# theovincent/iS-DQN

Hardware: AMD Instinct MI355X
Metric: gradient-steps/sec (batch=256, K=9, 84x84x4) (higher is better)
Workload: dtype bf16x3 (split-bf16 MFMA operands hi+lo, fp32 accumulate)

## Files before the change

is-dqn_amd/csrc/gemm_core.h:

```cpp
#pragma once
#include <cstdio>
#include <cstdlib>
#include <type_traits>
#include "common.h"

namespace isdqn {

typedef __attribute__((ext_vector_type(8))) __bf16 bf16x8;
typedef __attribute__((ext_vector_type(4))) short s16x4;
typedef __attribute__((ext_vector_type(8))) short s16x8;
typedef __attribute__((ext_vector_type(4))) float f32x4;

constexpr int GEMM_BK = 32;
constexpr int GEMM_THREADS = 256;

__device__ __forceinline__ int xcd_remap(int bid, int n_blocks) {
    const int xcd = bid & 7, q = n_blocks >> 3, r = n_blocks & 7;
    const int base = xcd < r ? xcd * (q + 1) : r * (q + 1) + (xcd - r) * q;
    return base + (bid >> 3);
}

#define LDS_AS __attribute__((address_space(3)))

__device__ __forceinline__ void split8(const float (&v)[8], bf16x8& hi, bf16x8& lo) {
// ... 86 lines not shown
    return ((chunk >> 4) << 2) + (((chunk >> 2) & 1) << 1) + ((chunk >> 3) & 1);
}
__device__ __forceinline__ constexpr int tr_row(int kk) {
    return 16 * (kk >> 4) + 8 * ((kk >> 2) & 1) + 2 * (kk & 3) + ((kk >> 3) & 1);
}
template <int ROWS, bool TR, int TR_PAD = 16>
struct TileGeom {
    static constexpr int PITCH = TR ? (ROWS + TR_PAD) : (GEMM_BK + 16);
    static constexpr int ELEMS = TR ? GEMM_BK * PITCH : ROWS * PITCH;
    static constexpr int CHUNKS = ROWS * (GEMM_BK / 8);
    static constexpr int PER_THREAD = (CHUNKS + GEMM_THREADS - 1) / GEMM_THREADS;
};

__device__ __forceinline__ void mfma_init(f32x4& acc) { acc = f32x4{0.f, 0.f, 0.f, 0.f}; }
__device__ __forceinline__ void mfma_acc(f32x4& acc, const bf16x8& a, const bf16x8& b) {
    acc = __builtin_amdgcn_mfma_f32_16x16x32_bf16(a, b, acc, 0, 0, 0);
}

template <bool TR, int PITCH>
__device__ __forceinline__ bf16x8 read_frag(const __bf16* tile, int row0, int lane) {
    if constexpr (!TR) {
        return *reinterpret_cast<const bf16x8*>(tile + (row0 + (lane & 15)) * PITCH + (lane >> 4) * 8);
    } else {
        const int g = lane >> 4, i = lane & 15, q = i >> 2, p = i & 3;
        const __bf16* a0 = tile + (16 * (g >> 1) + 2 * q + (g & 1)) * PITCH + row0 + 4 * p;
        const __bf16* a1 = a0 + 8 * PITCH;
        s16x4 lo = __builtin_amdgcn_ds_read_tr16_b64_v4i16((LDS_AS s16x4*)a0);
        s16x4 hi = __builtin_amdgcn_ds_read_tr16_b64_v4i16((LDS_AS s16x4*)a1);
        s16x8 r = __builtin_shufflevector(lo, hi, 0, 1, 2, 3, 4, 5, 6, 7);
        return __builtin_bit_cast(bf16x8, r);
    }
}

template <class P, class = void>
struct KGroupsOf { static constexpr int value = 1; };
template <class P>
struct KGroupsOf<P, std::void_t<decltype(P::KG)>> { static constexpr int value = P::KG; };
template <class P, class = void>
struct TrPadAOf { static constexpr int value = 16; };
template <class P>
struct TrPadAOf<P, std::void_t<decltype(P::TR_PAD_A)>> { static constexpr int value = P::TR_PAD_A; };
template <class P, class = void>
struct TrPadBOf { static constexpr int value = 16; };
template <class P>
struct TrPadBOf<P, std::void_t<decltype(P::TR_PAD_B)>> { static constexpr int value = P::TR_PAD_B; };
template <class P, class = void>
struct AS8Of { static constexpr bool value = false; };
template <class P>
struct AS8Of<P, std::void_t<decltype(P::A_S8)>> { static constexpr bool value = P::A_S8; };
template <class P, class = void>
struct BS8Of { static constexpr bool value = false; };
template <class P>
struct BS8Of<P, std::void_t<decltype(P::B_S8)>> { static constexpr bool value = P::B_S8; };

template <class P>
struct GemmTraits {
    static constexpr int BM = P::BM, BN = P::BN, WM = P::WM, WN = P::WN;
    static constexpr int MT = BM / WM / 16, NT = BN / WN / 16;
    static constexpr int PASSES = P::PASSES;
    static constexpr int A_PLANES = PASSES >= 2 ? 2 : 1;
    static constexpr int B_PLANES = PASSES >= 3 ? 2 : 1;
    using GA = TileGeom<BM, P::A_TR, TrPadAOf<P>::value>;
    using GB = TileGeom<BN, P::B_TR, TrPadBOf<P>::value>;
    static constexpr int STAGE_ELEMS = A_PLANES * GA::ELEMS + B_PLANES * GB::ELEMS;
    static constexpr int KG = KGroupsOf<P>::value;
    static constexpr int PIPE_BYTES = KG * 2 * STAGE_ELEMS * 2;
    static constexpr int XCHG_BYTES = KG > 1 ? KG * 4 * NT * 4 * 64 * 4 : 0;
    static constexpr int EPI_BYTES = P::EPI_LDS_BYTES + XCHG_BYTES;
    static constexpr int LDS_BYTES = PIPE_BYTES > EPI_BYTES ? PIPE_BYTES : EPI_BYTES;
};

template <class P>
__global__ __launch_bounds__(GEMM_THREADS * KGroupsOf<P>::value) void gemm_kernel(const P p) {
    ISDQN_EMPTY_KERNEL_RETURN
    using T = GemmTraits<P>;
    constexpr int KG = T::KG;
    using GA = typename T::GA;
    using GB = typename T::GB;
    constexpr int MT = T::MT, NT = T::NT, PASSES = T::PASSES;
    extern __shared__ __attribute__((aligned(16))) char smem_raw[];
    __bf16* smem = reinterpret_cast<__bf16*>(smem_raw);

    typename P::Tile tile;
    if (!p.tile((int)blockIdx.x, tile)) return;

    const int kg = KG > 1 ? (int)threadIdx.x / GEMM_THREADS : 0;
    const int tid = (int)threadIdx.x - kg * GEMM_THREADS;
    const int lane = tid & 63;
    const int wave = tid >> 6;
    const int wm = wave / P::WN, wn = wave % P::WN;
    const int wave_m = wm * (MT * 16), wave_n = wn * (NT * 16);

    typename P::ACtx actx[GA::PER_THREAD];
    typename P::BCtx bctx[GB::PER_THREAD];
    int a_lds[GA::PER_THREAD], a_var[GA::PER_THREAD];
    int b_lds[GB::PER_THREAD], b_var[GB::PER_THREAD];
    bool a_on[GA::PER_THREAD], b_on[GB::PER_THREAD];
#pragma unroll
    for (int i = 0; i < GA::PER_THREAD; ++i) {
        int c = tid + i * GEMM_THREADS;
        a_on[i] = c < GA::CHUNKS;
        if (!a_on[i]) c = 0;
        if constexpr (!P::A_TR) {
            int r = stash_row(c), kc = c & 3;
            actx[i] = p.a_ctx(tile, tile.m0 + r);
            a_var[i] = kc * 8;
            a_lds[i] = r * GA::PITCH + kc * 8;
        } else {
            int kk = c / (T::BM / 8), rc = c % (T::BM / 8);
            actx[i] = p.a_ctx(tile, tile.m0 + rc * 8);
            a_var[i] = kk;
            a_lds[i] = tr_row(kk) * GA::PITCH + rc * 8;
        }
    }
#pragma unroll
    for (int i = 0; i < GB::PER_THREAD; ++i) {
        int c = tid + i * GEMM_THREADS;
        b_on[i] = c < GB::CHUNKS;
        if (!b_on[i]) c = 0;
        if constexpr (!P::B_TR) {
            int r = stash_row(c), kc = c & 3;
            bctx[i] = p.b_ctx(tile, tile.n0 + r);
            b_var[i] = kc * 8;
            b_lds[i] = r * GB::PITCH + kc * 8;
        } else {
            int kk = c / (T::BN / 8), rc = c % (T::BN / 8);
            bctx[i] = p.b_ctx(tile, tile.n0 + rc * 8);
            b_var[i] = kk;
            b_lds[i] = tr_row(kk) * GB::PITCH + rc * 8;
        }
    }

    float sa[GA::PER_THREAD][8], sb[GB::PER_THREAD][8];

    auto fetch = [&](int k) {
#pragma unroll
        for (int i = 0; i < GA::PER_THREAD; ++i)
// ... 31 lines not shown
                chunk_hi<BS8Of<P>::value>(sb[i], hi);
            }
            *reinterpret_cast<bf16x8*>(b_hi + b_lds[i]) = hi;
        }
    };

    f32x4 acc[MT][NT];
#pragma unroll
    for (int mt = 0; mt < MT; ++mt)
#pragma unroll
        for (int nt = 0; nt < NT; ++nt) mfma_init(acc[mt][nt]);

    auto compute = [&](int stage) {
        const __bf16* base = smem + (kg * 2 + stage) * T::STAGE_ELEMS;
        const __bf16* a_hi = base;
        const __bf16* a_lo = base + GA::ELEMS;
        const __bf16* b_hi = base + T::A_PLANES * GA::ELEMS;
        const __bf16* b_lo = b_hi + GB::ELEMS;
        bf16x8 fa_hi[MT], fa_lo[MT];
#pragma unroll
        for (int mt = 0; mt < MT; ++mt) {
            fa_hi[mt] = read_frag<P::A_TR, GA::PITCH>(a_hi, wave_m + mt * 16, lane);
            if constexpr (PASSES >= 2) fa_lo[mt] = read_frag<P::A_TR, GA::PITCH>(a_lo, wave_m + mt * 16, lane);
        }
#pragma unroll
        for (int nt = 0; nt < NT; ++nt) {
            bf16x8 fb_hi = read_frag<P::B_TR, GB::PITCH>(b_hi, wave_n + nt * 16, lane);
            bf16x8 fb_lo;
            if constexpr (PASSES >= 3) fb_lo = read_frag<P::B_TR, GB::PITCH>(b_lo, wave_n + nt * 16, lane);
#pragma unroll
            for (int mt = 0; mt < MT; ++mt) {
                if constexpr (PASSES >= 3)
                    mfma_acc(acc[mt][nt], fa_hi[mt], fb_lo);
                if constexpr (PASSES >= 2)
                    mfma_acc(acc[mt][nt], fa_lo[mt], fb_hi);
                mfma_acc(acc[mt][nt], fa_hi[mt], fb_hi);
            }
        }
    };

    const int nsteps = ((tile.k1 - tile.k0 + GEMM_BK - 1) / GEMM_BK + KG - 1) / KG;
    if (nsteps > 0) {
        fetch(tile.k0 + kg * GEMM_BK);
        stash(0);
        __syncthreads();
        for (int s = 0; s < nsteps; ++s) {
            const bool more = s + 1 < nsteps;
            if (more) fetch(tile.k0 + ((s + 1) * KG + kg) * GEMM_BK);
            compute(s & 1);
            if (more) stash((s + 1) & 1);
            __syncthreads();
        }
    }
    if constexpr (KG > 1) {
        static_assert(KG == 2 && MT == 2, "one row tile per K group");
        float* red = reinterpret_cast<float*>(smem_raw + P::EPI_LDS_BYTES);
#pragma unroll
        for (int nt = 0; nt < NT; ++nt)
#pragma unroll
            for (int r = 0; r < 4; ++r) {
                const float give = kg == 0 ? acc[1][nt][r] : acc[0][nt][r];
                red[(((kg * 4 + wave) * NT + nt) * 4 + r) * 64 + lane] = give;
            }
        __syncthreads();
        f32x4 mine[1][NT];
#pragma unroll
        for (int nt = 0; nt < NT; ++nt)
#pragma unroll
            for (int r = 0; r < 4; ++r) {
                const float got = red[((((1 - kg) * 4 + wave) * NT + nt) * 4 + r) * 64 + lane];
                mine[0][nt][r] = (kg == 0 ? acc[0][nt][r] : acc[1][nt][r]) + got;
            }
        p.epilogue(tile, mine, tile.m0 + wave_m + kg * 16, tile.n0 + wave_n, lane, smem_raw);
    } else {
        p.epilogue(tile, acc, tile.m0 + wave_m, tile.n0 + wave_n, lane, smem_raw);
    }
}

template <class P>
static int launch_gemm(const P& p, int n_blocks, hipStream_t stream) {
    using T = GemmTraits<P>;
    static LdsConfigured configured;
    int rc = ensure_dynamic_lds(&gemm_kernel<P>, T::LDS_BYTES, configured);
    if (rc) return rc;
    ISDQN_REPORT_OCCUPANCY((&gemm_kernel<P>), GEMM_THREADS * T::KG, T::LDS_BYTES, n_blocks);
    if (n_blocks <= 0) return ISDQN_OK;
    hipLaunchKernelGGL(gemm_kernel<P>, dim3(n_blocks), dim3(GEMM_THREADS * T::KG), T::LDS_BYTES, stream, p);
    ISDQN_HIP_CHECK(hipGetLastError());
    return ISDQN_OK;
}

__device__ __forceinline__ void zero8(float (&v)[8]) {
#pragma unroll
    for (int i = 0; i < 8; ++i) v[i] = 0.f;
}
__device__ __forceinline__ float row16_sum(float x) {
    auto dpp = [](float v, auto ctrl) {
        return __builtin_bit_cast(float, __builtin_amdgcn_update_dpp(0, __builtin_bit_cast(int, v), decltype(ctrl)::value, 0xF, 0xF, true));
    };
    x += dpp(x, std::integral_constant<int, 0xB1>{});
    x += dpp(x, std::integral_constant<int, 0x4E>{});
    x += dpp(x, std::integral_constant<int, 0x124>{});
    x += dpp(x, std::integral_constant<int, 0x128>{});
    return x;
}

// ... 85 lines not shown
```

is-dqn_amd/csrc/head_chain.h:

```cpp
#pragma once
struct HeadChainParams {
    const float* slabs;
    int n_slabs;
    int64_t slab_stride, row_pitch;
    const float* hbias;
    float* act;
    float* z;
    const float* W;
    const float* bias;
    const float* gamma;
    const float* beta;
    int B, S, F, Fp, O, Op, K, A, oh;
    const int* action;
    const float* reward;
    const uint8_t* terminal;
    const float* loss_weights;
    const float* discount;
    float gamma_n, huber_delta;
    int double_q;
    Munchausen mu;
    float* dout;
    float* dz;
    float* part;
    float* q_values;
    float* targets;
    double* priorities;
    float* loss_part;
    float* dbh_part;
    int* adam_count;
    float b1, b2;
    float* adam_consts;
    long long* stamps;
};

constexpr int HC_MAX_COLS = 4;
constexpr int HC_THREADS = 512, HC_WAVES = HC_THREADS / 64;
constexpr int HC_KU = 16 / HC_WAVES;

__host__ __device__ inline int head_chain_pitch(int Fp) { return (Fp + 31) / 32 * 32 + 8; }
static inline int head_chain_lds_bytes(int Fp, int Op, int K, int passes, int S) {
    const int PA = head_chain_pitch(Fp);
    return (passes >= 2 ? 2 : 1) * 16 * PA * 2 + (HC_WAVES * 16 * Op + 16 * Op + S * Op + Op + 4 + 2 * S * Fp) * 4 + S * K * 12 +
           HC_WAVES * 2 * S * 2 * 4 + 64;
}

template <int PASSES, int COLS, int SMAX>
__global__ __launch_bounds__(HC_THREADS) void head_chain_kernel(const HeadChainParams p) {
    ISDQN_EMPTY_KERNEL_RETURN
    extern __shared__ __attribute__((aligned(16))) char hc_smem[];
    const int PA = head_chain_pitch(p.Fp);
    constexpr int A_PLANES = PASSES >= 2 ? 2 : 1;
    __bf16* a_hi = reinterpret_cast<__bf16*>(hc_smem);
    __bf16* a_lo = a_hi + 16 * PA;
    float* qpart = reinterpret_cast<float*>(a_hi + A_PLANES * 16 * PA);
    float* s_q = qpart + HC_WAVES * 16 * p.Op;
    float* s_dq = s_q + 16 * p.Op;
    float* s_d = s_dq + SMAX * p.Op;
    float* s_td = s_d + SMAX * p.K;
    float* s_wtd = s_td + SMAX * p.K;
    float* s_red = s_wtd + SMAX * p.K;
    float* s_bias = s_red + HC_WAVES * 2 * SMAX * 2;
// ... 7 lines not shown
        if ((i) == 0) p.stamps[(int64_t)blockIdx.x * 8 + 7] = (long long)__builtin_amdgcn_s_memrealtime(); \
    }
#else
#define HC_STAMP(i)
#endif
    HC_STAMP(0);
    const int S = p.S, b0 = (int)blockIdx.x * S;
    const int Fp = p.Fp, Op = p.Op, K = p.K, A = p.A;

    if (blockIdx.x == 0 && tid == 0) {
        int t = *p.adam_count + 1;
        *p.adam_count = t;
        p.adam_consts[0] = (float)(1.0 - pow_int((double)p.b1, t));
        p.adam_consts[1] = (float)(1.0 - pow_int((double)p.b2, t));
    }

    int act[SMAX];
#pragma unroll
    for (int s = 0; s < SMAX; ++s) {
        ISDQN_BOUNDS_CHECK((s < S && b0 + s < p.B) ? (const void*)(p.action + b0 + s) : zero_chunk(), 4, 20);
        act[s] = *(const ISDQN_GLOBAL int*)((s < S && b0 + s < p.B) ? (const void*)(p.action + b0 + s) : zero_chunk());
    }
    float td_r, td_w, td_g;
    uint8_t td_term;
    {
        const int s = tid / K;
        const bool ok = tid < S * K && b0 + s < p.B;
        const bool okw = ok && p.loss_weights != nullptr;
        ISDQN_BOUNDS_CHECK(okw ? (const void*)(p.loss_weights + b0 + s) : zero_chunk(), 4, 29);
        td_w = *(const ISDQN_GLOBAL float*)(okw ? (const void*)(p.loss_weights + b0 + s) : zero_chunk());
        const bool okg = ok && p.discount != nullptr;
        ISDQN_BOUNDS_CHECK(okg ? (const void*)(p.discount + b0 + s) : zero_chunk(), 4, 50);
        td_g = *(const ISDQN_GLOBAL float*)(okg ? (const void*)(p.discount + b0 + s) : zero_chunk());
        ISDQN_BOUNDS_CHECK(ok ? (const void*)(p.reward + b0 + s) : zero_chunk(), 4, 21);
        ISDQN_BOUNDS_CHECK(ok ? (const void*)(p.terminal + b0 + s) : zero_chunk(), 1, 22);
        td_r = *(const ISDQN_GLOBAL float*)(ok ? (const void*)(p.reward + b0 + s) : zero_chunk());
        td_term = *(const ISDQN_GLOBAL uint8_t*)(ok ? (const void*)(p.terminal + b0 + s) : zero_chunk());
    }
    ISDQN_BOUNDS_CHECK(tid < p.O ? (const void*)(p.bias + tid) : zero_chunk(), 4, 23);
    const float bias_v = *(const ISDQN_GLOBAL float*)(tid < p.O ? (const void*)(p.bias + tid) : zero_chunk());
    float ga[COLS], be[COLS];
#pragma unroll
    for (int j = 0; j < COLS; ++j) {
        const int c = tid + j * HC_THREADS;
        const bool ok = p.gamma != nullptr && c < p.F;
        ISDQN_BOUNDS_CHECK(ok ? (const void*)(p.gamma + c) : zero_chunk(), 4, 24);
        ISDQN_BOUNDS_CHECK(ok ? (const void*)(p.beta + c) : zero_chunk(), 4, 24);
        ga[j] = *(const ISDQN_GLOBAL float*)(ok ? (const void*)(p.gamma + c) : zero_chunk());
        be[j] = *(const ISDQN_GLOBAL float*)(ok ? (const void*)(p.beta + c) : zero_chunk());
    }

    constexpr int R2 = 2 * SMAX;
    constexpr int TPR = HC_THREADS / R2;
    constexpr int SB = 32;
    static_assert(TPR % 64 == 0, "a wave must not straddle two rows");
    float m1 = 0.f, m2 = 0.f;
    {
        const int r = tid / TPR, q = tid - r * TPR;
        const int smp = r < S ? r : r - S;
        const bool row_ok = r < 2 * S && b0 + smp < p.B;
        const int64_t grow = r < S ? (int64_t)(b0 + smp) : (int64_t)p.B + b0 + smp;
        for (int c0 = q * 4; c0 < Fp; c0 += TPR * 4) {
            float hb4[4];
#pragma unroll
            for (int e = 0; e < 4; ++e) {
                ISDQN_BOUNDS_CHECK(c0 + e < p.F ? (const void*)(p.hbias + c0 + e) : zero_chunk(), 4, 25);
                hb4[e] = *(const ISDQN_GLOBAL float*)(c0 + e < p.F ? (const void*)(p.hbias + c0 + e) : zero_chunk());
            }
            const ISDQN_GLOBAL f32x4* base = (const ISDQN_GLOBAL f32x4*)(row_ok ? (const void*)(p.slabs + grow * p.row_pitch + c0) : zero_chunk());
            const int64_t strd = row_ok ? p.slab_stride / 4 : 0;
            f32x4 sum = f32x4{0.f, 0.f, 0.f, 0.f};
            for (int s0 = 0; s0 < p.n_slabs; s0 += SB) {
                f32x4 t[SB];
#pragma unroll
                for (int u = 0; u < SB; ++u) {
                    ISDQN_BOUNDS_CHECK((const void*)(base + min(s0 + u, p.n_slabs - 1) * strd), 16, 26);
                    t[u] = base[min(s0 + u, p.n_slabs - 1) * strd];
                }
#pragma unroll
                for (int u = 0; u < SB; ++u)
                    if (s0 + u < p.n_slabs) sum += t[u];
            }
            float v[4];
#pragma unroll
            for (int e = 0; e < 4; ++e) {
                v[e] = c0 + e < p.F ? sum[e] + hb4[e] : 0.f;
                m1 += v[e];
                m2 += v[e] * v[e];
            }
            *reinterpret_cast<float4*>(s_pre + r * Fp + c0) = make_float4(v[0], v[1], v[2], v[3]);
        }
    }

    HC_STAMP(6);
    const int nkt = (PA - 8) / 32, NT = (Op + 15) / 16;
    const int nks = (nkt + 15) / 16, n_items = ((NT + 1) / 2) * nks;
    const int kg8 = (lane >> 4) * 8;
    const int arow = (lane & 15) * PA + kg8;
    auto issue_w = [&](float (&v)[2][HC_KU][8], int item) {
        const int pair = item / nks, ksb = wave + 16 * (item - pair * nks);
#pragma unroll
        for (int t = 0; t < 2; ++t)
#pragma unroll
            for (int u = 0; u < HC_KU; ++u) {
                const int o = (pair * 2 + t) * 16 + (lane & 15), ks = ksb + HC_WAVES * u;
                const bool ok = item < n_items && o < p.O && ks < nkt && ks * 32 + kg8 < Fp;
                load8_aligned(ok ? p.W + (int64_t)o * Fp + ks * 32 + kg8 : zero_chunk(), v[t][u]);
            }
    };
    float wv0[2][HC_KU][8], wv1[2][HC_KU][8];
    issue_w(wv0, 0);

    float zv[SMAX][COLS];
    {
        for (int off = 32; off > 0; off >>= 1) {
            m1 += __shfl_xor(m1, off);
            m2 += __shfl_xor(m2, off);
        }
        if (lane == 0) {
            s_red[wave * 2] = m1;
            s_red[wave * 2 + 1] = m2;
        }
        __syncthreads();
        constexpr int WPR = TPR / 64;
#pragma unroll
        for (int r = 0; r < R2; ++r) {
            float a1 = s_red[r * WPR * 2], a2 = s_red[r * WPR * 2 + 1];
#pragma unroll
            for (int w = 1; w < WPR; ++w) {
                a1 += s_red[(r * WPR + w) * 2];
                a2 += s_red[(r * WPR + w) * 2 + 1];
            }
            const float mean = a1 / (float)p.F;
            const float rstd = rsqrtf(fmaxf(a2 / (float)p.F - mean * mean, 0.f) + 1e-6f);
            const int smp = r < S ? r : r - S;
            const bool row_ok = r < 2 * S && b0 + smp < p.B;
            const int64_t grow = r < S ? (int64_t)(b0 + smp) : (int64_t)p.B + b0 + smp;
#pragma unroll
            for (int j = 0; j < COLS; ++j) {
                const int c = tid + j * HC_THREADS;
                const float v = c < Fp ? s_pre[r * Fp + c] : 0.f;
                float y = v;
                if (p.gamma != nullptr && c < p.F) y = (v - mean) * (rstd * ga[j]) + be[j];
                y = fmaxf(y, 0.f);
                if (c >= p.F) y = 0.f;
                if (row_ok && c < Fp) {
                    s8_store_elem(p.act + grow * Fp, c, y);
                    if (r < S) p.z[grow * Fp + c] = v;
                }
                if (r < 2 * S && c < PA - 8) {
                    const float ys = row_ok ? y : 0.f;
                    const __bf16 h = (__bf16)ys;
                    a_hi[r * PA + c] = h;
                    if constexpr (PASSES >= 2) a_lo[r * PA + c] = (__bf16)(ys - (float)h);
                }
                if (r < SMAX) zv[r < SMAX ? r : 0][j] = (row_ok && r < S && c < p.F) ? v : 0.f;
            }
        }
    }
    for (int i = tid; i < SMAX * Op; i += HC_THREADS) s_dq[i] = 0.f;
    if (tid < Op) s_bias[tid] = bias_v;
    for (int o = tid + HC_THREADS; o < Op; o += HC_THREADS) s_bias[o] = o < p.O ? p.bias[o] : 0.f;
    __syncthreads();
    HC_STAMP(1);

    {
        f32x4 acc[2];
        auto run_item = [&](float (&v)[2][HC_KU][8], int item) {
            const int pair = item / nks, ksi = item - pair * nks, ksb = wave + 16 * ksi;
            if (ksi == 0) {
                acc[0] = acc[1] = f32x4{0.f, 0.f, 0.f, 0.f};
            }
#pragma unroll
            for (int u = 0; u < HC_KU; ++u) {
                const int ks = min(ksb + HC_WAVES * u, nkt - 1);
                const bf16x8 ah = *reinterpret_cast<const bf16x8*>(a_hi + arow + ks * 32);
                bf16x8 al;
                if constexpr (PASSES >= 2) al = *reinterpret_cast<const bf16x8*>(a_lo + arow + ks * 32);
#pragma unroll
                for (int t = 0; t < 2; ++t) {
                    bf16x8 bh, bl;
                    if constexpr (PASSES >= 2) {
                        split8(v[t][u], bh, bl);
                        if constexpr (PASSES >= 3)
                            mfma_acc(acc[t], ah, bl);
                        mfma_acc(acc[t], al, bh);
                    } else {
                        round8(v[t][u], bh);
                    }
                    mfma_acc(acc[t], ah, bh);
                }
            }
            const bool last = ksi + 1 == nks;
            if (last) {
#pragma unroll
                for (int t = 0; t < 2; ++t) {
                    const int o = (pair * 2 + t) * 16 + (lane & 15);
                    if (o < Op) {
#pragma unroll
                        for (int r = 0; r < 4; ++r) qpart[(wave * 16 + (lane >> 4) * 4 + r) * Op + o] = acc[t][r];
                    }
                }
            }
        };
        for (int item = 0; item < n_items; item += 2) {
            issue_w(wv1, item + 1);
            run_item(wv0, item);
            issue_w(wv0, item + 2);
            if (item + 1 < n_items) run_item(wv1, item + 1);
        }
    }

    auto issue_rows = [&](float (&w)[SMAX][4][COLS], int k0) {
#pragma unroll
        for (int s = 0; s < SMAX; ++s)
#pragma unroll
            for (int u = 0; u < 4; ++u) {
                const bool on = s < S && k0 + u < K;
                const float* wr = p.W + (int64_t)(on ? (p.oh + k0 + u) * A + act[s] : 0) * Fp;
#pragma unroll
                for (int j = 0; j < COLS; ++j) {
                    const int c = tid + j * HC_THREADS;
                    ISDQN_BOUNDS_CHECK(wr + (c < p.F ? c : 0), 4, 27);
                    w[s][u][j] = *(const ISDQN_GLOBAL float*)(wr + (c < p.F ? c : 0));
                }
            }
    };
    HC_STAMP(2);
    float wr0[SMAX][4][COLS], wr1[SMAX][4][COLS];
    issue_rows(wr0, 0);
    __syncthreads();
    for (int i = tid; i < 2 * S * Op; i += HC_THREADS) {
        const int o = i % Op;
        float v = qpart[i];
#pragma unroll
        for (int w = 1; w < HC_WAVES; ++w) v += qpart[w * 16 * Op + i];
        s_q[i] = o < p.O ? v + s_bias[o] : 0.f;
    }
    __syncthreads();

    const float inv_b = 1.f / (float)p.B;
// ... 191 lines not shown
```

is-dqn_amd/csrc/learn_step.h:

```cpp
#pragma once
struct SideStream {
    hipStream_t stream = nullptr;
    hipEvent_t ev[2 * MAX_LAYERS + 4];
    int n_ev = 0;
    std::atomic<unsigned> next{0};
    std::atomic<int> state{0};
};
static SideStream* side_stream() {
    static SideStream per_dev[ISDQN_MAX_DEVICES];
    if (ISDQN_DEV_ENV("ISDQN_SINGLE_STREAM")) return nullptr;
    SideStream& s = per_dev[current_device_slot()];
    int st = s.state.load(std::memory_order_acquire);
    if (st == 2) return &s;
    if (st == -1) return nullptr;
    int expected = 0;
    if (s.state.compare_exchange_strong(expected, 1)) {
        bool ok = hipStreamCreateWithFlags(&s.stream, hipStreamNonBlocking) == hipSuccess;
        s.n_ev = 2 * MAX_LAYERS + 4;
        for (int i = 0; ok && i < s.n_ev; ++i) ok = hipEventCreateWithFlags(&s.ev[i], hipEventDisableTiming) == hipSuccess;
        s.state.store(ok ? 2 : -1, std::memory_order_release);
        return ok ? &s : nullptr;
    }
    while ((st = s.state.load(std::memory_order_acquire)) == 1) {}
    return st == 2 ? &s : nullptr;
// ... 41 lines not shown
        c.hc_wg = n_wg;
    }
}

static int learn_forward(const LearnCtx& c) {
    const Plan& P = c.P;
    const isdqn_batch* batch = c.batch;
    float* ws = c.ws;
    const int B = c.B;
    int rc;
    if (c.target_params != nullptr) {
        struct Form {
            NetInput t_in; int t_rows; float* t_out; int expect_rows;
            NetInput on_in; int on_rows;
        };
        const int stack = c.cfg->arch != ISDQN_ARCH_FC ? c.cfg->obs_c : 0;
        const NetInput nx{batch->frames, batch->frame_stride, batch->frame_ids, 0, batch->next_state, nullptr, 0, 2 * stack, stack};
        const NetInput on{batch->frames, batch->frame_stride, batch->frame_ids, 0, batch->state, nullptr, 0, 2 * stack, 0};
        const Form f =
            c.munchausen ? Form{c.in, P.N2, ws + P.out_t_off, P.N2, on, B}
            : c.double_q ? Form{nx, B, ws + P.out_t_off, B, c.in, P.N2}
                         : Form{nx, B, ws + P.out_off + (int64_t)B * P.nlog_p, 0, on, B};
        rc = refresh_mirror(P, c.target_params, ws, c.st);
        if (rc) return rc;
        rc = net_forward(P, c.x3, c.target_params, f.t_in, f.t_rows, 0, ws, f.t_out, c.st);
        if (rc) return rc;
        if (f.expect_rows > 0 && P.head_nb > 0) {
            rc = head_expect_rows(P, ws + P.logits_t_off, f.expect_rows, ws + P.qt_off, c.st);
            if (rc) return rc;
        }
        rc = refresh_mirror(P, c.params, ws, c.st);
        if (rc) return rc;
        return net_forward(P, c.x3, c.params, f.on_in, f.on_rows, B, ws, ws + P.out_off, c.st);
    }
    if (!(batch->flags & ISDQN_BATCH_MIRROR_CURRENT)) {
        rc = refresh_mirror(P, c.params, ws, c.st);
        if (rc) return rc;
    }
    return net_forward(P, c.x3, c.params, c.in, P.N2, B, ws, ws + P.out_off, c.st, c.hc_S ? P.n_layers - 1 : -1, c.hc_S ? P.n_layers - 2 : -1);
}

static int launch_head_chain(const LearnCtx& c) {
    const Plan& P = c.P;
    const Layer &hid = c.hid(), &head = c.head();
    float* ws = c.ws;
    HeadChainParams hp;
    hp.act = ws + hid.act_off; hp.z = ws + hid.z_off;
    hp.slabs = ws + P.slab_off;
    hp.n_slabs = effective_splits(hid.in_unpadded_ld ? hid.in_f : hid.K, hid.fwd_splits);
    hp.slab_stride = hid.out_p;
    hp.row_pitch = (int64_t)hp.n_slabs * hid.out_p;
    hp.hbias = c.params + hid.b_off;
    hp.W = c.params + head.w_off; hp.bias = c.params + head.b_off;
    hp.gamma = hid.has_ln ? c.params + hid.g_off : nullptr;
    hp.beta = hid.has_ln ? c.params + hid.be_off : nullptr;
    hp.B = c.B; hp.S = c.hc_S; hp.F = hid.out_f; hp.Fp = hid.out_p; hp.O = P.nha; hp.Op = P.nha_p; hp.K = c.K; hp.oh = P.oh;
    hp.A = P.n_actions;
    hp.action = c.batch->action; hp.reward = c.batch->reward; hp.terminal = c.batch->terminal;
    hp.loss_weights = c.batch->loss_weights; hp.discount = batch_discount(c.batch);
    hp.gamma_n = c.cfg->gamma_n; hp.huber_delta = c.cfg->huber_delta;
    hp.double_q = c.double_q ? 1 : 0;
    hp.mu = Munchausen{c.cfg->munchausen_tau, c.cfg->munchausen_alpha, c.cfg->munchausen_clip};
    hp.dout = ws + P.dout_off; hp.dz = ws + hid.dz_off; hp.part = ws + hid.part_off;
    hp.q_values = c.q_values; hp.targets = c.targets; hp.priorities = c.priorities;
    hp.loss_part = ws + P.lpart_off; hp.dbh_part = hp.loss_part + (int64_t)c.hc_wg * c.K;
    hp.adam_count = c.adam_count; hp.b1 = c.cfg->adam_b1; hp.b2 = c.cfg->adam_b2; hp.adam_consts = ws + P.adam_tab_off;
    hp.stamps = stamps_for("head_chain");
    const int lds = head_chain_lds_bytes(hid.out_p, P.nha_p, c.K, c.x3 ? 3 : 1, c.hc_S);
    const int cols = ceil_div(hid.out_p, HC_THREADS) <= 1 ? 1 : ceil_div(hid.out_p, HC_THREADS) <= 2 ? 2 : 4;
    auto launch_hc = [&](auto kern, int slot) -> int {
        static LdsConfigured configured[18];
        if (int rc2 = ensure_dynamic_lds(kern, lds, configured[slot])) return rc2;
        ISDQN_REPORT_OCCUPANCY(kern, HC_THREADS, lds, c.hc_wg);
        hipLaunchKernelGGL(kern, dim3(c.hc_wg), dim3(HC_THREADS), lds, c.st, hp);
        ISDQN_HIP_CHECK(hipGetLastError());
        return ISDQN_OK;
    };
    auto by_cols = [&](auto passes_c, auto s_c, int base) -> int {
        constexpr int PS = decltype(passes_c)::value, SS = decltype(s_c)::value;
        return cols == 1 ? launch_hc(&head_chain_kernel<PS, 1, SS>, base) : cols == 2 ? launch_hc(&head_chain_kernel<PS, 2, SS>, base + 1)
                                                                        : launch_hc(&head_chain_kernel<PS, 4, SS>, base + 2);
    };
    auto by_s = [&](auto passes_c, int base) -> int {
        return c.hc_S == 1 ? by_cols(passes_c, std::integral_constant<int, 1>{}, base)
             : c.hc_S == 2 ? by_cols(passes_c, std::integral_constant<int, 2>{}, base + 3)
                           : by_cols(passes_c, std::integral_constant<int, 4>{}, base + 6);
    };
    return c.x3 ? by_s(std::integral_constant<int, 3>{}, 0) : by_s(std::integral_constant<int, 1>{}, 9);
}

static int head_chain_sums(const LearnCtx& c, hipStream_t s) {
    return loss_finalize(c.P, c.cfg, c.ws, c.hc_wg, c.K, c.P.nha_p, c.losses, c.loss_accum, true, nullptr, s);
}
static int head_chain_tail(const LearnCtx& c, hipStream_t s) {
    if (int rc = head_chain_sums(c, s)) return rc;
    const Layer& head = c.head();
    return dense_wgrad(head, c.x3, c.in, c.ws + c.hid().act_off, c.ws + c.P.dout_off, c.P.nlog_p, c.ws + head.gw_off, c.B, s);
}

static int learn_loss(const LearnCtx& c) {
    const bool tnet = (c.double_q || c.munchausen) && c.target_params != nullptr;
    if (!c.hc_S) {
        int rc = loss_and_finalize(c.P, c, c.double_q, tnet ? c.ws + c.P.out_t_off + (c.munchausen ? (int64_t)c.B * c.P.nlog_p : 0) : nullptr,
                                   (tnet && c.munchausen) ? c.ws + c.P.out_t_off : nullptr);
        if (rc || !(c.learn() && c.P.dueling)) return rc;
        const Plan& P = c.P;
// ... 107 lines not shown
    int fork_after_dgrad(WgradJob& job, bool* defer) {
        if (!fork_late) {
            if (int rc = chain(c.ss, c.st, job.stream)) return rc;
            if (int rc = signal_priorities()) return rc;
            forked = true;
            return run_head_tail(job.stream);
        }
        if (head_event != nullptr && head_pending) {
            ISDQN_HIP_CHECK(hipStreamWaitEvent(job.stream, head_event, 0));
            if (int rc = run_head_tail(job.stream)) return rc;
        }
        job.wait = next_event(c.ss);
        ISDQN_HIP_CHECK(hipEventRecord(job.wait, c.st));
        *defer = true;
        forked = true;
        return signal_priorities();
    }
    int chain_layer0() {
        if (int rc = chain(c.ss, c.st, c.wst)) return rc;
        forked = layer0_chained = true;
        return run_head_tail(c.wst);
    }
    int flush() {
        if (deferred.layer < 0) return ISDQN_OK;
        const WgradJob j = deferred;
        deferred.layer = -1;
        ISDQN_HIP_CHECK(hipStreamWaitEvent(j.stream, j.wait, 0));
        if (int rc = run_head_tail(j.stream)) return rc;
        return weight_gradient(c, j, adam);
    }
    int finish() {
        if (int rc = flush()) return rc;
        if (int rc = run_head_tail(c.st)) return rc;
        return signal_priorities();
    }
};

static bool dense_dgrad_ln_applies(const Layer& l, const Layer& below, int B) {
    return l.kind == 1 && below.kind != 1 && below.cout_p == 64 && !l.in_unpadded_ld && below.part_rows >= ceil_div(B, 128) * below.npix;
}
static int dense_dgrad_ln(const LearnCtx& c, const Layer& l, const Layer& below, const float* dz, int dz_ld, ReduceJobs* red) {
    float* ws = c.ws;
    const int B = c.B;
    auto launch = [&](auto prob) {
        prob.A = MatSrc{dz, dz_ld, B, l.out_p, 1};
        prob.B = MatSrc{c.wmir() + l.w_off, l.in_p, l.out_f, l.in_p, 1};
        prob.z = ws + below.z_off;
        prob.gamma = below.has_ln ? c.params + below.g_off : nullptr;
        prob.beta = below.has_ln ? c.params + below.be_off : nullptr;
        prob.dz_out = ws + below.dz_off;
        prob.part = ws + below.part_off;
        prob.ldc = l.in_p; prob.M = B; prob.N = l.in_p; prob.K = l.out_p; prob.c_in = below.out_f;
        prob.tiles_m = ceil_div(B, decltype(prob)::BM); prob.tiles_n = l.in_p / 64;
        return launch_gemm(prob, prob.tiles_m * prob.tiles_n, c.st);
    };
    static const bool no_kg = ISDQN_DEV_ENV("ISDQN_NO_KGROUPS");
    const bool kg2 = !no_kg && ceil_div(B, 128) * (l.in_p / 64) <= 256 && l.out_p % 64 == 0;
    int rc;
#if defined(ISDQN_DGRAD64)
    (void)kg2;
    rc = c.x3 ? launch(DenseDgradLN<3, 64>{}) : launch(DenseDgradLN<1, 64>{});
    constexpr int DG_BM = 64;
#else
    if (kg2) rc = c.x3 ? launch(DenseDgradLN<3, 128, 2>{}) : launch(DenseDgradLN<1, 128, 2>{});
    else rc = c.x3 ? launch(DenseDgradLN<3, 128>{}) : launch(DenseDgradLN<1, 128>{});
    constexpr int DG_BM = 128;
#endif
    if (rc) return rc;
    add_reduce_job(*red, ws + below.part_off, ceil_div(B, DG_BM) * (l.in_p / 64), 3 * below.out_p, ws + below.red_off);
    return ISDQN_OK;
}

static int data_gradient(const LearnCtx& c, int i, const float* dz, int dz_ld, bool* dz_fused, ReduceJobs* red) {
    const Layer &l = c.P.L[i], &below = c.P.L[i - 1];
    float* da = c.ws + c.P.da_off;
    *dz_fused = false;
    if (l.is_head && c.hc_S) return ISDQN_OK;
    if (l.kind == 0) {
        int rc = conv_dgrad_img(l, below, c.x3, c.params, c.wmir(), dz, c.ws, c.B, c.st, dz_fused, red);
        if (rc || *dz_fused) return rc;
        return conv_dgrad(l, c.x3, c.wmir(), dz, da, c.B, c.st);
    }
    if (dense_dgrad_ln_applies(l, below, c.B)) {
        *dz_fused = true;
        return dense_dgrad_ln(c, l, below, dz, dz_ld, red);
    }
    const bool narrow = ceil_div(c.B, 128) * ceil_div(l.in_p, 128) < 200;
    return dense_dgrad(l, c.x3, c.wmir(), dz, dz_ld, da, c.B, narrow, c.st);
}

static int learn_backward(const LearnCtx& c, BackwardSchedule& sched, AdamList* adam, ReduceJobs* red) {
    const Plan& P = c.P;
    float* ws = c.ws;
    const int B = c.B;
    int rc;
    const float* dz_cur = ws + (P.dueling ? P.dout_raw_off : P.dout_off);
    int dz_ld = P.dueling ? P.raw_p : P.nlog_p;
    bool dz_fused = false;
    for (int i = P.n_layers - 1; i >= 0; --i) {
        const Layer& l = P.L[i];
        if (l.is_head) {
            adam[c.hc_S && c.ss ? 1 : 0].add(l.b_off, l.out_p, ws + (P.dueling ? P.dbh_raw_off : P.dbh_off), 1, 0, c.wd(2));
        } else {
            dz_cur = ws + l.dz_off;
            dz_ld = l.out_p;
            if (c.hc_S && i == P.n_layers - 2) {
// ... 197 lines not shown
```

is-dqn_amd/csrc/net_problems.h:

```cpp
#pragma once
#include "gemm_core.h"

namespace isdqn {

struct FrameSrc {
    const uint8_t* frames;
    int64_t stride;
    const int* ids;
    int stack;
    int paired_B;
    int H, W;
    int id_pitch = 0, id_off = 0;
    __device__ __forceinline__ int frame_id(int j, int c) const {
#if defined(ISDQN_DEV)
        if (ids == nullptr) return j * stack + c;
#endif
        if (paired_B > 0) {
            const int* q = j < paired_B ? ids + (int64_t)j * 2 * stack + c : ids + (int64_t)(j - paired_B) * 2 * stack + stack + c;
            ISDQN_BOUNDS_CHECK(q, 4, 4);
            return *q;
        }
        ISDQN_BOUNDS_CHECK(ids + (int64_t)j * (id_pitch ? id_pitch : stack) + id_off + c, 4, 4);
        return ids[(int64_t)j * (id_pitch ? id_pitch : stack) + id_off + c];
    }
// ... 149 lines not shown
                }
                if (adam.wd != 0.f) {
#pragma unroll
                    for (int r = 0; r < 4; ++r) np[r] = adamw_decay(np[r], pp[it][r], adam.lr, adam.wd);
                }
                if (on[it] && adam.grad_out) *reinterpret_cast<float4*>(adam.grad_out + off[it]) = g;
                if (on[it] && adam.update) {
#if !defined(ISDQN_NO_STREAMING)
                    __builtin_nontemporal_store(nm, (ISDQN_GLOBAL f32x4*)(adam.m + off[it]));
                    __builtin_nontemporal_store(nv, (ISDQN_GLOBAL f32x4*)(adam.v + off[it]));
                    __builtin_nontemporal_store(np, (ISDQN_GLOBAL f32x4*)(adam.p + off[it]));
#else
                    *reinterpret_cast<f32x4*>(adam.m + off[it]) = nm;
                    *reinterpret_cast<f32x4*>(adam.v + off[it]) = nv;
                    *reinterpret_cast<f32x4*>(adam.p + off[it]) = np;
#endif
                    s8_store_quad(adam.mirror, (int)off[it], np[0], np[1], np[2], np[3]);
                }
            }
            return;
        }
        float* c = C + (int64_t)t.split * slab_stride;
#pragma unroll
        for (int mt = 0; mt < MT; ++mt)
#pragma unroll
            for (int nt = 0; nt < NT; ++nt) {
                int col = n_wave + nt * 16 + (lane & 15);
#pragma unroll
                for (int r = 0; r < 4; ++r) {
                    int row = m_wave + mt * 16 + (lane >> 4) * 4 + r;
                    if (row < M && col < N) c[(int64_t)row * ldc + col] = acc[mt][nt][r];
                }
            }
    }
};

template <int PASSES_, int BM_ = 128, int KG_ = 1>
struct DenseDgradLN {
    static constexpr int BM = BM_, BN = 64, WM = 4, WN = 1, PASSES = PASSES_;
    static constexpr int KG = KG_;
    static constexpr bool A_TR = false, B_TR = true;
    static constexpr bool A_S8 = true;
    static constexpr bool B_S8 = true;
    static constexpr int TR_PITCH = 68;
    static constexpr int SP_BYTES = 4 * KG_ * 3 * 64 * 4;
    static constexpr int EPI_LDS_BYTES = SP_BYTES + 4 * KG_ * 16 * TR_PITCH * 4;
    MatSrc A, B;
    const float* z;
    const float *gamma, *beta;
    float* dz_out;
    float* part;
    int ldc, M, N, K, c_in;
    int tiles_m, tiles_n;
    struct Tile { int m0, n0, k0, k1, wg; };
    struct ACtx { int fixed; };
    struct BCtx { int fixed; };
    __device__ __forceinline__ bool tile(int bid, Tile& t) const {
        t.wg = bid;
        bid = xcd_remap(bid, tiles_m * tiles_n);
        t.m0 = (bid % tiles_m) * BM;
        t.n0 = (bid / tiles_m) * BN;
        t.k0 = 0; t.k1 = K;
        return bid < tiles_m * tiles_n;
    }
    __device__ __forceinline__ ACtx a_ctx(const Tile&, int fixed) const { return ACtx{fixed}; }
    __device__ __forceinline__ BCtx b_ctx(const Tile&, int fixed) const { return BCtx{fixed}; }
    __device__ __forceinline__ void load_a(const Tile&, const ACtx& c, int var, float (&v)[8]) const { A.load(c.fixed, var, v); }
    __device__ __forceinline__ void load_b(const Tile&, const BCtx& c, int var, float (&v)[8]) const { B.load(var, c.fixed, v); }
    template <int MT, int NT>
    __device__ __forceinline__ void epilogue(const Tile& t, f32x4 (&acc)[MT][NT], int m_wave, int n_wave, int lane, char* smem) const {
        static_assert(NT == 4, "one wave must hold all 64 channels of a row");
        const int grp = lane >> 4, li = lane & 15, wave = (m_wave - t.m0) / (MT * 16);
        float ga[NT], be[NT], dg[NT], db[NT], dbias[NT];
#pragma unroll
        for (int nt = 0; nt < NT; ++nt) {
            const int ch = nt * 16 + li;
            const bool ok = ch < c_in;
            ga[nt] = (ok && gamma) ? gamma[ch] : 1.f;
            be[nt] = (ok && gamma) ? beta[ch] : 0.f;
            dg[nt] = db[nt] = dbias[nt] = 0.f;
        }
        const float inv_c = 1.f / (float)c_in;
        float* tr = reinterpret_cast<float*>(smem + SP_BYTES) + wave * 16 * TR_PITCH;
        float zall[MT][4][NT];
#pragma unroll
        for (int mt = 0; mt < MT; ++mt)
#pragma unroll
            for (int r = 0; r < 4; ++r) {
                const int row = m_wave + mt * 16 + grp * 4 + r;
                const int64_t base = (int64_t)(row < M ? row : 0) * ldc + t.n0;
#pragma unroll
                for (int nt = 0; nt < NT; ++nt) {
                    ISDQN_BOUNDS_CHECK(z + base + nt * 16 + li, 4, 11);
                    zall[mt][r][nt] = *(const ISDQN_GLOBAL float*)(z + base + nt * 16 + li);
                }
            }
#pragma unroll
        for (int mt = 0; mt < MT; ++mt)
#pragma unroll
            for (int r = 0; r < 4; ++r) {
                const int row = m_wave + mt * 16 + grp * 4 + r;
                const bool row_ok = row < M;
                const int64_t base = (int64_t)(row_ok ? row : 0) * ldc + t.n0;
                float zv[NT];
#pragma unroll
                for (int nt = 0; nt < NT; ++nt) zv[nt] = zall[mt][r][nt];
                float out[NT];
                if (gamma != nullptr) {
                    float s1 = 0.f, s2 = 0.f;
#pragma unroll
                    for (int nt = 0; nt < NT; ++nt) {
                        const bool ok = (nt * 16 + li) < c_in;
                        s1 += ok ? zv[nt] : 0.f;
                        s2 += ok ? zv[nt] * zv[nt] : 0.f;
                    }
                    s1 = row16_sum(s1);
                    s2 = row16_sum(s2);
                    const float mean = s1 * inv_c;
                    const float rstd = rsqrtf(fmaxf(s2 * inv_c - mean * mean, 0.f) + 1e-6f);
                    float xh[NT], gg[NT], m1 = 0.f, m2 = 0.f;
#pragma unroll
                    for (int nt = 0; nt < NT; ++nt) {
                        const bool ok = row_ok && (nt * 16 + li) < c_in;
                        xh[nt] = (zv[nt] - mean) * rstd;
                        const float y = xh[nt] * ga[nt] + be[nt];
                        const float dy = (ok && y > 0.f) ? acc[mt][nt][r] : 0.f;
                        dg[nt] += dy * xh[nt];
                        db[nt] += dy;
                        gg[nt] = dy * ga[nt];
                        m1 += gg[nt];
                        m2 += gg[nt] * xh[nt];
                    }
                    m1 = row16_sum(m1);
                    m2 = row16_sum(m2);
                    m1 *= inv_c;
                    m2 *= inv_c;
#pragma unroll
                    for (int nt = 0; nt < NT; ++nt) {
                        const bool ok = row_ok && (nt * 16 + li) < c_in;
                        out[nt] = ok ? rstd * (gg[nt] - m1 - xh[nt] * m2) : 0.f;
                        dbias[nt] += out[nt];
                    }
                } else {
#pragma unroll
                    for (int nt = 0; nt < NT; ++nt) {
                        const bool ok = row_ok && (nt * 16 + li) < c_in;
                        out[nt] = (ok && zv[nt] > 0.f) ? acc[mt][nt][r] : 0.f;
                        dbias[nt] += out[nt];
                    }
                }
#pragma unroll
                for (int nt = 0; nt < NT; ++nt) tr[(grp * 4 + r) * TR_PITCH + nt * 16 + li] = out[nt];
                if (r == 3) {
#pragma unroll
                    for (int u = 0; u < 2; ++u) {
                        const int chunk = lane + u * 64, rl = chunk >> 3, c8 = (chunk & 7) * 8;
                        const int orow = m_wave + mt * 16 + rl;
                        float v[8];
                        const f32x4 lo4 = *reinterpret_cast<const f32x4*>(tr + rl * TR_PITCH + c8);
                        const f32x4 hi4 = *reinterpret_cast<const f32x4*>(tr + rl * TR_PITCH + c8 + 4);
                        v[0] = lo4[0]; v[1] = lo4[1]; v[2] = lo4[2]; v[3] = lo4[3];
                        v[4] = hi4[0]; v[5] = hi4[1]; v[6] = hi4[2]; v[7] = hi4[3];
                        if (orow < M) s8_store_group(dz_out + (int64_t)orow * ldc + t.n0 + c8, v);
                    }
                }
            }
        float* sp = reinterpret_cast<float*>(smem);
#pragma unroll
        for (int nt = 0; nt < NT; ++nt) {
            dg[nt] += __shfl_xor(dg[nt], 16); dg[nt] += __shfl_xor(dg[nt], 32);
            db[nt] += __shfl_xor(db[nt], 16); db[nt] += __shfl_xor(db[nt], 32);
            dbias[nt] += __shfl_xor(dbias[nt], 16); dbias[nt] += __shfl_xor(dbias[nt], 32);
            if (grp == 0) {
                sp[(wave * 3 + 0) * 64 + nt * 16 + li] = dg[nt];
                sp[(wave * 3 + 1) * 64 + nt * 16 + li] = db[nt];
                sp[(wave * 3 + 2) * 64 + nt * 16 + li] = dbias[nt];
            }
        }
        __syncthreads();
        const int tid = threadIdx.x;
        if (tid < 3 * 64) {
            const int which = tid / 64, c = tid % 64;
            float sum = sp[(0 * 3 + which) * 64 + c];
#pragma unroll
            for (int w = 1; w < 4 * KG; ++w) sum += sp[(w * 3 + which) * 64 + c];
            part[((int64_t)t.wg * 3 + which) * 64 + c] = sum;
        }
    }
};

struct ConvGeom {
    int hin, win, cin_p, hout, wout, cout, cout_p, ksz, stride, pad, npix, K;
    int stride_sh;
    FastDiv d_npix, d_wout, d_cinp, d_ksz, d_coutp;
};

template <int BM_, int PASSES_, bool U8>
struct ConvFwd {
    static constexpr int BM = BM_, BN = 128, WM = 1, WN = 4, PASSES = PASSES_;
    static constexpr bool A_TR = false, B_TR = false;
    static constexpr bool A_S8 = true;
    static constexpr bool B_S8 = !U8;
    static constexpr int EPI_LDS_BYTES = 0;
    ConvGeom g;
    MatSrc W;
    const float* in;
    FrameSrc fs;
    const float *bias, *gamma, *beta;
    float scale;
    float* act;
    float* z;
    int n_pix_total, z_pix;
    struct Tile { int m0, n0, k0, k1; };
    struct ACtx { int row; };
    struct BCtx { int j, iy0, ix0, valid, f0, f1, f2, f3; };
    __device__ __forceinline__ bool tile(int bid, Tile& t) const {
        t.m0 = 0; t.n0 = bid * BN; t.k0 = 0; t.k1 = g.K;
        return t.n0 < n_pix_total;
    }
    __device__ __forceinline__ ACtx a_ctx(const Tile&, int row) const { return ACtx{row}; }
    __device__ __forceinline__ void load_a(const Tile&, const ACtx& c, int k, float (&v)[8]) const { W.load(c.row, k, v); }
    __device__ __forceinline__ BCtx b_ctx(const Tile&, int pix) const {
        BCtx c;
        c.valid = pix < n_pix_total;
        uint32_t j, p, oy, ox;
        g.d_npix.divmod(c.valid ? pix : 0, j, p);
        g.d_wout.divmod(p, oy, ox);
        c.j = (int)j;
        c.iy0 = (int)oy * g.stride - g.pad;
        c.ix0 = (int)ox * g.stride - g.pad;
        c.f0 = c.f1 = c.f2 = c.f3 = -1;
        if constexpr (U8) {
            c.f0 = fs.frame_id(c.j, 0);
            if (fs.stack > 1) c.f1 = fs.frame_id(c.j, 1);
            if (fs.stack > 2) c.f2 = fs.frame_id(c.j, 2);
            if (fs.stack > 3) c.f3 = fs.frame_id(c.j, 3);
        }
        return c;
    }
    __device__ __forceinline__ void load_b(const Tile&, const BCtx& c, int k, float (&v)[8]) const {
// ... 235 lines not shown
```

Measured before the change: 4359.

## Read pre-split head weights, shrink slab batch, add dev-only GEMM timestamps

```diff
diff --git a/is-dqn_amd/csrc/gemm_core.h b/is-dqn_amd/csrc/gemm_core.h
--- a/is-dqn_amd/csrc/gemm_core.h
+++ b/is-dqn_amd/csrc/gemm_core.h
@@ -162,6 +162,25 @@
 struct BS8Of { static constexpr bool value = false; };
 template <class P>
 struct BS8Of<P, std::void_t<decltype(P::B_S8)>> { static constexpr bool value = P::B_S8; };
+
+#if defined(ISDQN_DEV)
+template <class P, class = void>
+struct HasStamps { static constexpr bool value = false; };
+template <class P>
+struct HasStamps<P, std::void_t<decltype(P::stamps)>> { static constexpr bool value = true; };
+template <class P>
+__device__ __forceinline__ void gemm_stamp(const P& p, int i) {
+    if constexpr (HasStamps<P>::value) {
+        if (p.stamps != nullptr && threadIdx.x == 0) {
+            p.stamps[(int64_t)blockIdx.x * 8 + i] = (long long)__builtin_amdgcn_s_memtime();
+            if (i == 0) p.stamps[(int64_t)blockIdx.x * 8 + 7] = (long long)__builtin_amdgcn_s_memrealtime();
+        }
+    }
+}
+#define ISDQN_GEMM_STAMP(p, i) gemm_stamp(p, i)
+#else
+#define ISDQN_GEMM_STAMP(p, i)
+#endif
 
 template <class P>
 struct GemmTraits {
@@ -193,6 +212,7 @@
 
     typename P::Tile tile;
     if (!p.tile((int)blockIdx.x, tile)) return;
+    ISDQN_GEMM_STAMP(p, 0);
 
     const int kg = KG > 1 ? (int)threadIdx.x / GEMM_THREADS : 0;
     const int tid = (int)threadIdx.x - kg * GEMM_THREADS;
@@ -330,6 +350,7 @@
             __syncthreads();
         }
     }
+    ISDQN_GEMM_STAMP(p, 1);
     if constexpr (KG > 1) {
         static_assert(KG == 2 && MT == 2, "one row tile per K group");
         float* red = reinterpret_cast<float*>(smem_raw + P::EPI_LDS_BYTES);
diff --git a/is-dqn_amd/csrc/head_chain.h b/is-dqn_amd/csrc/head_chain.h
--- a/is-dqn_amd/csrc/head_chain.h
+++ b/is-dqn_amd/csrc/head_chain.h
@@ -7,6 +7,7 @@
     float* act;
     float* z;
     const float* W;
+    const float* Wm;
     const float* bias;
     const float* gamma;
     const float* beta;
@@ -120,7 +121,7 @@
 
     constexpr int R2 = 2 * SMAX;
     constexpr int TPR = HC_THREADS / R2;
-    constexpr int SB = 32;
+    constexpr int SB = 16;
     static_assert(TPR % 64 == 0, "a wave must not straddle two rows");
     float m1 = 0.f, m2 = 0.f;
     {
@@ -139,15 +140,17 @@
             const int64_t strd = row_ok ? p.slab_stride / 4 : 0;
             f32x4 sum = f32x4{0.f, 0.f, 0.f, 0.f};
             for (int s0 = 0; s0 < p.n_slabs; s0 += SB) {
+                const int rem = p.n_slabs - s0;
                 f32x4 t[SB];
 #pragma unroll
-                for (int u = 0; u < SB; ++u) {
-                    ISDQN_BOUNDS_CHECK((const void*)(base + min(s0 + u, p.n_slabs - 1) * strd), 16, 26);
-                    t[u] = base[min(s0 + u, p.n_slabs - 1) * strd];
-                }
-#pragma unroll
                 for (int u = 0; u < SB; ++u)
-                    if (s0 + u < p.n_slabs) sum += t[u];
+                    if (u < rem) {
+                        ISDQN_BOUNDS_CHECK((const void*)(base + (s0 + u) * strd), 16, 26);
+                        t[u] = base[(s0 + u) * strd];
+                    }
+#pragma unroll
+                for (int u = 0; u < SB; ++u)
+                    if (u < rem) sum += t[u];
             }
             float v[4];
 #pragma unroll
@@ -173,7 +176,8 @@
             for (int u = 0; u < HC_KU; ++u) {
                 const int o = (pair * 2 + t) * 16 + (lane & 15), ks = ksb + HC_WAVES * u;
                 const bool ok = item < n_items && o < p.O && ks < nkt && ks * 32 + kg8 < Fp;
-                load8_aligned(ok ? p.W + (int64_t)o * Fp + ks * 32 + kg8 : zero_chunk(), v[t][u]);
+                ISDQN_BOUNDS_CHECK(ok ? p.Wm + (int64_t)o * Fp + ks * 32 + kg8 : zero_chunk(), 32, 58);
+                load8_aligned(ok ? p.Wm + (int64_t)o * Fp + ks * 32 + kg8 : zero_chunk(), v[t][u]);
             }
     };
     float wv0[2][HC_KU][8], wv1[2][HC_KU][8];
@@ -249,12 +253,12 @@
                 for (int t = 0; t < 2; ++t) {
                     bf16x8 bh, bl;
                     if constexpr (PASSES >= 2) {
-                        split8(v[t][u], bh, bl);
+                        s8_unpack(v[t][u], bh, bl);
                         if constexpr (PASSES >= 3)
                             mfma_acc(acc[t], ah, bl);
                         mfma_acc(acc[t], al, bh);
                     } else {
-                        round8(v[t][u], bh);
+                        s8_unpack_hi(v[t][u], bh);
                     }
                     mfma_acc(acc[t], ah, bh);
                 }
diff --git a/is-dqn_amd/csrc/learn_step.h b/is-dqn_amd/csrc/learn_step.h
--- a/is-dqn_amd/csrc/learn_step.h
+++ b/is-dqn_amd/csrc/learn_step.h
@@ -117,6 +117,7 @@
     hp.row_pitch = (int64_t)hp.n_slabs * hid.out_p;
     hp.hbias = c.params + hid.b_off;
     hp.W = c.params + head.w_off; hp.bias = c.params + head.b_off;
+    hp.Wm = c.wmir() + head.w_off;
     hp.gamma = hid.has_ln ? c.params + hid.g_off : nullptr;
     hp.beta = hid.has_ln ? c.params + hid.be_off : nullptr;
     hp.B = c.B; hp.S = c.hc_S; hp.F = hid.out_f; hp.Fp = hid.out_p; hp.O = P.nha; hp.Op = P.nha_p; hp.K = c.K; hp.oh = P.oh;
@@ -330,6 +331,9 @@
         prob.part = ws + below.part_off;
         prob.ldc = l.in_p; prob.M = B; prob.N = l.in_p; prob.K = l.out_p; prob.c_in = below.out_f;
         prob.tiles_m = ceil_div(B, decltype(prob)::BM); prob.tiles_n = l.in_p / 64;
+#if defined(ISDQN_DEV)
+        prob.stamps = stamps_for("dgrad_ln");
+#endif
         return launch_gemm(prob, prob.tiles_m * prob.tiles_n, c.st);
     };
     static const bool no_kg = ISDQN_DEV_ENV("ISDQN_NO_KGROUPS");
diff --git a/is-dqn_amd/csrc/net_problems.h b/is-dqn_amd/csrc/net_problems.h
--- a/is-dqn_amd/csrc/net_problems.h
+++ b/is-dqn_amd/csrc/net_problems.h
@@ -225,6 +225,9 @@
     float* part;
     int ldc, M, N, K, c_in;
     int tiles_m, tiles_n;
+#if defined(ISDQN_DEV)
+    long long* stamps;
+#endif
     struct Tile { int m0, n0, k0, k1, wg; };
     struct ACtx { int fixed; };
     struct BCtx { int fixed; };
@@ -268,6 +271,10 @@
                     zall[mt][r][nt] = *(const ISDQN_GLOBAL float*)(z + base + nt * 16 + li);
                 }
             }
+#if defined(ISDQN_DEV)
+        if (stamps != nullptr) asm volatile("s_waitcnt vmcnt(0)" ::: "memory");
+#endif
+        ISDQN_GEMM_STAMP(*this, 2);
 #pragma unroll
         for (int mt = 0; mt < MT; ++mt)
 #pragma unroll
@@ -338,6 +345,7 @@
                     }
                 }
             }
+        ISDQN_GEMM_STAMP(*this, 3);
         float* sp = reinterpret_cast<float*>(smem);
 #pragma unroll
         for (int nt = 0; nt < NT; ++nt) {
@@ -359,6 +367,7 @@
             for (int w = 1; w < 4 * KG; ++w) sum += sp[(w * 3 + which) * 64 + c];
             part[((int64_t)t.wg * 3 + which) * 64 + c] = sum;
         }
+        ISDQN_GEMM_STAMP(*this, 4);
     }
 };
 
```

Result: no change. 4390 (median of 6 runs) (+0.7%).
